# michael-fonder/M4Depth

Measured on AMD Instinct MI355X. Metric: frames/s, higher is better.
Workload: dtype f32

## Files before the change

include/m4depth_hip.h:

```cpp
#ifndef M4DEPTH_HIP_H_
#define M4DEPTH_HIP_H_

#include <stdint.h>

#ifdef __cplusplus
extern "C" {
#endif

#define M4D_ABI_VERSION 6

int m4d_abi_version(void);
long long m4d_launch_count(void);
const char* m4d_build_info(void);


int m4d_backproject_fwd(const float* input, const float* coords, const int dims[6],
                        float* out, void* stream);

int m4d_backproject_bwd(const float* grad, const float* input, const float* coords,
                        const int dims[6], float* input_grad, float* coords_grad, void* stream);


int m4d_dense_image_warp(const float* image, const float* flow, int B, int H, int W, int C,
                         float* out, int32_t* index_out, void* stream);
// ... 196 lines not shown

int m4d_level_post(const float* refiner_out, const float* rot, int rot_c, const float* trans,
                   const float* cam_f, const float* cam_c, int b, int h, int w, float scale,
                   float* parallax, float* depth, float* other, float* depth_state, void* stream);

int m4d_bias_act(const float* x, const float* bias, long long rows, int C, float slope,
                 float* out, void* stream);

int m4d_bias_act_padded(const float* x, const float* bias, int b, int h, int w, int C, float slope,
                        float* out, int out_h, int out_w, int off_y, int off_x, void* stream);

int m4d_conv3x3_bias_act(const float* x, const float* wp, const float* bias, int b, int h, int w,
                         int Cin, int Cout, int CoutPad, float slope, float* out, void* stream);
long long m4d_conv3x3_workspace_floats(int b, int h, int w, int CoutPad);
int m4d_conv3x3s_bias_act_ws(const float* x, const float* wp, const float* bias, int b, int h, int w,
                             int Cin, int Cout, int CoutPad, int stride, float slope, float* out,
                             float* workspace, long long workspace_floats, void* stream);
int m4d_conv3x3_bias_act_ws(const float* x, const float* wp, const float* bias, int b, int h, int w,
                            int Cin, int Cout, int CoutPad, float slope, float* out, float* workspace,
                            long long workspace_floats, void* stream);
int m4d_conv3x3s_bias_act_wsb(const float* x, const float* wp, const float* bias, int b, int split_batch, int h, int w,
                              int Cin, int Cout, int CoutPad, int stride, float slope, float* out,
                              float* workspace, long long workspace_floats, void* stream);
int m4d_conv3x3_lat(const float* x, int s_in, long long x_slab_floats, const float* x_bias, float x_slope,
                    const void* wp, const float* bias, int b, int h, int w, int Cin, int Cout, float slope,
                    int mt, int kw, int s_out, float* out, long long out_slab_floats, void* stream);
int m4d_conv3x3s_lat(const float* x, int s_in, long long x_slab_floats, const float* x_bias, float x_slope,
                     const void* wp, const float* bias, int b, int h, int w, int Cin, int Cout, int stride, float slope,
                     int mt, int kw, int s_out, float* out, long long out_slab_floats, void* stream);
int m4d_conv3x3_lat_f16(const float* x, int s_in, long long x_slab_floats, const float* x_bias, float x_slope,
                        const void* wp, const float* bias, int b, int h, int w, int Cin, int Cout, float slope,
                        int mt, int kw, int s_out, float* out, long long out_slab_floats, void* stream);
int m4d_partial_finish(const float* x, int s_in, long long x_slab_floats, const float* bias, float slope,
                       long long pixels, int C, float* out, void* stream);

int m4d_conv3x3_small_bias_act(const float* x, const float* wp, const float* bias, int b, int h, int w,
                               int Cin, int Cout, int CoutPad, float slope, float* out, void* stream);
int m4d_conv3x3s_small_bias_act(const float* x, const float* wp, const float* bias, int b, int h, int w,
                                int Cin, int Cout, int CoutPad, int stride, float slope, float* out, void* stream);
int m4d_conv3x3_small6_bias_act(const float* x, const void* wp6, const float* bias, int b, int h, int w,
                                int Cin, int Cout, int CoutPad, float slope, float* out, void* stream);

long long m4d_dinl_workspace_floats(int b, int C);
int m4d_dinl_fwd_padded(const float* x, const float* scale, const float* bias, int b, int h, int w, int C,
                        float slope, float* workspace, float* out, int out_h, int out_w, int off_y,
                        int off_x, void* stream);
int m4d_dinl_fwd(const float* x, const float* scale, const float* bias, int b, int h, int w, int C,
                 float slope, float* workspace, float* out, void* stream);

int m4d_enc_level0_fwd(const float* images, int bsz, long long stride_b, long long stride_t,
                       const float* w1_hwio, const float* bias1, const float* dn_scale, const float* dn_bias,
                       float dn_slope, const float* w2_hwio, const float* bias2, float slope,
                       int b, int h, int w, float* workspace, float* out, void* stream);
int m4d_enc_level0_stats(const float* images, int bsz, long long stride_b, long long stride_t,
                         const float* w1_hwio, const float* bias1, int b, int h, int w, float* workspace,
                         float* mean, float* var, void* stream);
int m4d_enc_level0_apply(const float* images, int bsz, long long stride_b, long long stride_t,
                         const float* w1_hwio, const float* bias1, const float* mean, const float* var,
                         const float* dn_scale, const float* dn_bias, float dn_slope, const float* w2_hwio,
                         const float* bias2, float slope, int b, int h, int w, float* out, void* stream);
int m4d_enc_head_fwd(const float* images, int bsz, long long stride_b, long long stride_t,
                     const float* w_hwio, const float* bias, int b, int h, int w, int C,
// ... 60 lines not shown
```

m4depth_amd/_lib.py:

```python
from __future__ import annotations

import ctypes
import os

import torch

_HERE = os.path.dirname(os.path.abspath(__file__))
LIB_FLAVOUR = os.environ.get("M4D_LIB_FLAVOUR", "product")
LIB_PATH = os.path.join(_HERE, "libm4depth_hip_exp.so" if LIB_FLAVOUR == "experiments" else "libm4depth_hip.so")

ABI_VERSION = 6

_c_fp = ctypes.c_void_p
_c_int = ctypes.c_int
_c_f = ctypes.c_float

class NormLevel(ctypes.Structure):
    _fields_ = [("x", ctypes.c_void_p), ("out", ctypes.c_void_p), ("pixels", ctypes.c_longlong), ("C", ctypes.c_int),
                ("nbre_cuts", ctypes.c_int)]


class ResetLevel(ctypes.Structure):
    _fields_ = [("features", ctypes.c_void_p), ("state_features", ctypes.c_void_p), ("depth_state", ctypes.c_void_p),
                ("parallax", ctypes.c_void_p), ("depth", ctypes.c_void_p), ("other", ctypes.c_void_p),
# ... 42 lines not shown
    "m4d_depth_export": [_c_fp, ctypes.c_longlong, _c_fp, ctypes.c_longlong, _c_fp, ctypes.c_longlong, _c_int, _c_int, _c_int,
                         _c_int, _c_fp, _c_int, ctypes.POINTER(_c_int), _c_fp, _c_f, _c_f, _c_f, _c_fp, _c_fp],
    "m4d_pose_accumulate": [_c_fp, _c_int, _c_fp, _c_fp, _c_int, _c_fp, _c_fp],
    "m4d_depth_cloud": [_c_fp, ctypes.c_longlong, _c_fp, ctypes.c_longlong, _c_fp, _c_fp, _c_fp, _c_int, _c_int, _c_int, _c_int,
                        _c_f, _c_f, _c_fp, _c_fp, _c_fp, _c_fp],
    "m4d_summary_images": [_c_int, ctypes.POINTER(ctypes.c_void_p), ctypes.POINTER(ctypes.c_longlong), ctypes.POINTER(_c_int),
                           ctypes.POINTER(_c_int), ctypes.POINTER(_c_int), ctypes.POINTER(_c_int),
                           ctypes.POINTER(ctypes.c_longlong), _c_int, _c_fp, _c_fp],
    "m4d_normalize_cuts": [_c_fp, _c_int, _c_int, _c_int, _c_int, _c_int, _c_fp, _c_fp],
    "m4d_resize_bilinear_v1": [_c_fp, _c_int, _c_int, _c_int, _c_int, _c_int, _c_int, _c_f, _c_fp, _c_fp],
    "m4d_resize_nearest": [_c_fp, _c_int, _c_int, _c_int, _c_int, _c_int, _c_int, _c_fp, _c_fp],
    "m4d_bias_act": [_c_fp, _c_fp, ctypes.c_longlong, _c_int, _c_f, _c_fp, _c_fp],
    "m4d_dinl_fwd": [_c_fp, _c_fp, _c_fp, _c_int, _c_int, _c_int, _c_int, _c_f, _c_fp, _c_fp, _c_fp],
    "m4d_dinl_fwd_padded": [_c_fp, _c_fp, _c_fp, _c_int, _c_int, _c_int, _c_int, _c_f, _c_fp, _c_fp,
                            _c_int, _c_int, _c_int, _c_int, _c_fp],
    "m4d_bias_act_padded": [_c_fp, _c_fp, _c_int, _c_int, _c_int, _c_int, _c_f, _c_fp, _c_int, _c_int, _c_int, _c_int, _c_fp],
    "m4d_conv3x3_bias_act": [_c_fp, _c_fp, _c_fp, _c_int, _c_int, _c_int, _c_int, _c_int, _c_int, _c_f, _c_fp, _c_fp],
    "m4d_conv3x3_bias_act_ws": [_c_fp, _c_fp, _c_fp, _c_int, _c_int, _c_int, _c_int, _c_int, _c_int, _c_f, _c_fp,
                                _c_fp, ctypes.c_longlong, _c_fp],
    "m4d_conv3x3s_bias_act_ws": [_c_fp, _c_fp, _c_fp, _c_int, _c_int, _c_int, _c_int, _c_int, _c_int, _c_int, _c_f,
                                 _c_fp, _c_fp, ctypes.c_longlong, _c_fp],
    "m4d_conv3x3s_bias_act_wsb": [_c_fp, _c_fp, _c_fp, _c_int, _c_int, _c_int, _c_int, _c_int, _c_int, _c_int, _c_int, _c_f,
                                  _c_fp, _c_fp, ctypes.c_longlong, _c_fp],
    "m4d_conv3x3_small_bias_act": [_c_fp, _c_fp, _c_fp, _c_int, _c_int, _c_int, _c_int, _c_int, _c_int, _c_f, _c_fp, _c_fp],
    "m4d_conv3x3s_small_bias_act": [_c_fp, _c_fp, _c_fp, _c_int, _c_int, _c_int, _c_int, _c_int, _c_int, _c_int, _c_f, _c_fp, _c_fp],
    "m4d_conv3x3_small6_bias_act": [_c_fp, _c_fp, _c_fp, _c_int, _c_int, _c_int, _c_int, _c_int, _c_int, _c_f, _c_fp, _c_fp],
    "m4d_conv3x3_lat": [_c_fp, _c_int, ctypes.c_longlong, _c_fp, _c_f, _c_fp, _c_fp, _c_int, _c_int, _c_int, _c_int, _c_int, _c_f,
                        _c_int, _c_int, _c_int, _c_fp, ctypes.c_longlong, _c_fp],
    "m4d_conv3x3s_lat": [_c_fp, _c_int, ctypes.c_longlong, _c_fp, _c_f, _c_fp, _c_fp, _c_int, _c_int, _c_int, _c_int, _c_int, _c_int,
                         _c_f, _c_int, _c_int, _c_int, _c_fp, ctypes.c_longlong, _c_fp],
    "m4d_conv3x3_lat_f16": [_c_fp, _c_int, ctypes.c_longlong, _c_fp, _c_f, _c_fp, _c_fp, _c_int, _c_int, _c_int, _c_int, _c_int,
                            _c_f, _c_int, _c_int, _c_int, _c_fp, ctypes.c_longlong, _c_fp],
    "m4d_partial_finish": [_c_fp, _c_int, ctypes.c_longlong, _c_fp, _c_f, ctypes.c_longlong, _c_int, _c_fp, _c_fp],
    "m4d_conv3x3_wino_bias_act": [_c_fp, _c_fp, _c_fp, _c_int, _c_int, _c_int, _c_int, _c_int, _c_int, _c_f, _c_fp, _c_fp],
    "m4d_conv3x3_wino2_bias_act": [_c_fp, _c_fp, _c_fp, _c_int, _c_int, _c_int, _c_int, _c_int, _c_int, _c_f, _c_fp, _c_fp],
    "m4d_conv3x3_wino6_bias_act": [_c_fp, _c_fp, _c_fp, _c_int, _c_int, _c_int, _c_int, _c_int, _c_int, _c_f, _c_fp, _c_fp],
    "m4d_conv3x3_wino6_bias_act_k": [_c_fp, _c_fp, _c_fp, _c_int, _c_int, _c_int, _c_int, _c_int, _c_int, _c_f, _c_fp, _c_int, _c_fp],
    "m4d_conv3x3_wino6_bias_act_ks": [_c_fp, _c_fp, _c_fp, _c_int, _c_int, _c_int, _c_int, _c_int, _c_int, _c_f, _c_fp, _c_int,
                                      _c_int, _c_int, _c_fp],
    "m4d_conv3x3_winof16_bias_act_ks": [_c_fp, _c_fp, _c_fp, _c_int, _c_int, _c_int, _c_int, _c_int, _c_int, _c_f, _c_fp,
                                        _c_int, _c_int, _c_fp],
    "m4d_enc_head_fwd": [_c_fp, _c_int, ctypes.c_longlong, ctypes.c_longlong, _c_fp, _c_fp, _c_int, _c_int, _c_int, _c_int,
                         _c_fp, _c_fp, _c_fp],
    "m4d_enc_level0_stats": [_c_fp, _c_int, ctypes.c_longlong, ctypes.c_longlong, _c_fp, _c_fp, _c_int, _c_int, _c_int, _c_fp, _c_fp, _c_fp,
                             _c_fp],
    "m4d_enc_level0_apply": [_c_fp, _c_int, ctypes.c_longlong, ctypes.c_longlong, _c_fp, _c_fp, _c_fp, _c_fp, _c_fp, _c_fp, _c_f, _c_fp,
                             _c_fp, _c_f, _c_int, _c_int, _c_int, _c_fp, _c_fp],
    "m4d_enc_level0_fwd": [_c_fp, _c_int, ctypes.c_longlong, ctypes.c_longlong, _c_fp, _c_fp, _c_fp, _c_fp, _c_f, _c_fp, _c_fp, _c_f,
# ... 171 lines not shown
```

m4depth_amd/csrc/m4d_conv.hip:

```cpp
#include <cstdlib>
#include "m4d_common.h"
#include "../../include/m4depth_hip.h"

namespace {

typedef float f32x16 __attribute__((ext_vector_type(16)));

struct ConvArgs {
  const float* x; const float* wp; const float* bias; float* out;
  int b, h, w, Cin, Cout, CoutPad, n_chunks, tiles_x, tiles_y;
  int oh, ow, pad_y, pad_x;
  float slope;
  int ksplit, chunks_per_split;
  float* ws;
  const float* dn_mean; const float* dn_var; const float* dn_scale; const float* dn_bias; float dn_slope;
  int ablate;
};

constexpr int kTW = 16, kTH = 8;
constexpr int kKC = 16, kRS = 20;

template <int NT, int TS, int STRIDE, bool DB, int MINB, bool DINL = false>
__global__ void __launch_bounds__(256, MINB)
conv3x3_mfma_kernel(const ConvArgs a) {
// ... 580 lines not shown
void dispatch_conv(const ConvArgs& a, int nt, dim3 grid, hipStream_t s) {
  const long long blocks = (long long)grid.x * grid.y * grid.z;
  static long long occ3_min_blocks = -1;
  if (occ3_min_blocks < 0) { const char* e = getenv("M4D_CONV_OCC3_MIN_BLOCKS"); occ3_min_blocks = e ? atoll(e) : 4 * 768; }
  switch (nt) {
    case 4:
      if (STRIDE == 1 && blocks >= occ3_min_blocks) launch_conv<4, 3, STRIDE, STRIDE == 1 ? 3 : 1>(a, grid, s);
      else launch_conv<4, 3, STRIDE, STRIDE == 1 ? 2 : 1>(a, grid, s);
      break;
    case 3: launch_conv<3, 3, STRIDE, STRIDE == 1 ? 3 : 2>(a, grid, s); break;
    case 2: launch_conv<2, STRIDE == 1 ? 9 : 3, STRIDE, STRIDE == 1 ? 3 : 2>(a, grid, s); break;
    default: launch_conv<1, 9, STRIDE, STRIDE == 1 ? 4 : 2>(a, grid, s); break;
  }
}

}

extern "C" int m4d_conv3x3_bias_act(const float* x, const float* wp, const float* bias, int b, int h, int w,
                                    int Cin, int Cout, int CoutPad, float slope, float* out, void* stream) {
  return m4d_conv3x3s_bias_act_ws(x, wp, bias, b, h, w, Cin, Cout, CoutPad, 1, slope, out, nullptr, 0, stream);
}

static int launch_conv3x3_small(const float* x, const float* wp, const float* bias, int b, int h, int w, int Cin, int Cout,
                                int CoutPad, int stride, float slope, float* out, void* stream) {
  M4D_CHECK_ARG(x && wp && bias && out && b > 0 && h > 0 && w > 0 && Cout > 0 && (stride == 1 || stride == 2));
  M4D_CHECK_ARG(Cin >= 16 && Cin % 4 == 0 && CoutPad % 32 == 0 && CoutPad >= Cout);
  M4D_CHECK_ARG(((((uintptr_t)x) | ((uintptr_t)wp)) & 15u) == 0);
  ConvArgs a;
  a.x = x; a.wp = wp; a.bias = bias; a.out = out; a.b = b; a.h = h; a.w = w; a.Cin = Cin; a.Cout = Cout;
  a.CoutPad = CoutPad; a.n_chunks = (Cin + kKC - 1) / kKC;
  a.dn_mean = a.dn_var = a.dn_scale = a.dn_bias = nullptr; a.dn_slope = 1.0f;
  a.ablate = 0; a.slope = slope;
  a.oh = (h + stride - 1) / stride; a.ow = (w + stride - 1) / stride;
  const int tot_y = (a.oh - 1) * stride + 3 - h, tot_x = (a.ow - 1) * stride + 3 - w;
  a.pad_y = (tot_y > 0 ? tot_y : 0) / 2; a.pad_x = (tot_x > 0 ? tot_x : 0) / 2;
  a.tiles_x = (a.ow + kSW - 1) / kSW; a.tiles_y = (a.oh + kSH - 1) / kSH;
  a.ksplit = 1; a.chunks_per_split = a.n_chunks; a.ws = nullptr;
  const int halo = ((kSW - 1) * stride + 3) * ((kSH - 1) * stride + 3);
  const size_t lds = (size_t)4 * (halo * kRS + kSB) * sizeof(float);
  if (stride == 1) M4D_LDS_OPT_IN(&conv3x3_small_kernel<1>);
  else M4D_LDS_OPT_IN(&conv3x3_small_kernel<2>);
  const dim3 grid((unsigned)(a.tiles_x * a.tiles_y), (unsigned)(CoutPad / 32), (unsigned)b);
  if (stride == 1) m4d_launch(conv3x3_small_kernel<1>, grid, dim3(256), lds, (hipStream_t)stream, a);
  else m4d_launch(conv3x3_small_kernel<2>, grid, dim3(256), lds, (hipStream_t)stream, a);
  return M4D_LAUNCH_RESULT();
}
extern "C" int m4d_conv3x3_small_bias_act(const float* x, const float* wp, const float* bias, int b, int h, int w,
                                          int Cin, int Cout, int CoutPad, float slope, float* out, void* stream) {
  return launch_conv3x3_small(x, wp, bias, b, h, w, Cin, Cout, CoutPad, 1, slope, out, stream);
}
extern "C" int m4d_conv3x3s_small_bias_act(const float* x, const float* wp, const float* bias, int b, int h, int w,
                                           int Cin, int Cout, int CoutPad, int stride, float slope, float* out, void* stream) {
  return launch_conv3x3_small(x, wp, bias, b, h, w, Cin, Cout, CoutPad, stride, slope, out, stream);
}

extern "C" int m4d_conv3x3_small6_bias_act(const float* x, const void* wp6, const float* bias, int b, int h, int w,
                                           int Cin, int Cout, int CoutPad, float slope, float* out, void* stream) {
  M4D_CHECK_ARG(x && wp6 && bias && out && b > 0 && h > 0 && w > 0 && Cout > 0);
  M4D_CHECK_ARG(Cin >= 16 && Cin % 4 == 0 && CoutPad % 32 == 0 && CoutPad >= Cout);
  M4D_CHECK_ARG(((((uintptr_t)x) | ((uintptr_t)wp6)) & 15u) == 0);
  ConvArgs a;
  a.x = x; a.wp = reinterpret_cast<const float*>(wp6); a.bias = bias; a.out = out; a.b = b; a.h = h; a.w = w; a.Cin = Cin; a.Cout = Cout;
  a.CoutPad = CoutPad; a.n_chunks = (Cin + kKC - 1) / kKC;
  a.dn_mean = a.dn_var = a.dn_scale = a.dn_bias = nullptr; a.dn_slope = 1.0f;
  a.ablate = 0; a.oh = h; a.ow = w; a.pad_y = a.pad_x = 1; a.slope = slope;
  a.tiles_x = (w + kSW - 1) / kSW; a.tiles_y = (h + kSH - 1) / kSH;
  a.ksplit = 1; a.chunks_per_split = a.n_chunks; a.ws = nullptr;
  constexpr size_t lds = (size_t)4 * (kS6A + kS6B) * sizeof(float);
  M4D_LDS_OPT_IN(&conv3x3_small6_kernel);
  m4d_launch(conv3x3_small6_kernel, dim3((unsigned)(a.tiles_x * a.tiles_y), (unsigned)(CoutPad / 32), (unsigned)b), dim3(256),
                     lds, (hipStream_t)stream, a);
  return M4D_LAUNCH_RESULT();
}

extern "C" long long m4d_conv3x3_workspace_floats(int b, int h, int w, int CoutPad) {
  return 32LL * b * h * w * CoutPad;
// ... 23 lines not shown
  a.dn_mean = mean; a.dn_var = var; a.dn_scale = dn_scale; a.dn_bias = dn_bias; a.dn_slope = dn_slope;
  constexpr int HP = ((kTW - 1) * 2 + 3) * ((kTH - 1) * 2 + 3);
  constexpr size_t lds = (size_t)(HP * kRS + 9 * 32 * kRS) * sizeof(float);
  if (lds > 64 * 1024) M4D_LDS_OPT_IN(&conv3x3_mfma_kernel<1, 9, 2, false, 2, true>);
  const dim3 grid((unsigned)(a.tiles_x * a.tiles_y), 1, (unsigned)b);
  m4d_launch((conv3x3_mfma_kernel<1, 9, 2, false, 2, true>), grid, dim3(256), lds, (hipStream_t)stream, a);
  return M4D_LAUNCH_RESULT();
}

extern "C" int m4d_conv3x3s_bias_act_wsb(const float* x, const float* wp, const float* bias, int b, int split_batch, int h,
                                         int w, int Cin, int Cout, int CoutPad, int stride, float slope, float* out,
                                         float* workspace, long long workspace_floats, void* stream);

extern "C" int m4d_conv3x3s_bias_act_ws(const float* x, const float* wp, const float* bias, int b, int h, int w,
                                        int Cin, int Cout, int CoutPad, int stride, float slope, float* out,
                                        float* workspace, long long workspace_floats, void* stream) {
  return m4d_conv3x3s_bias_act_wsb(x, wp, bias, b, b, h, w, Cin, Cout, CoutPad, stride, slope, out, workspace,
                                   workspace_floats, stream);
}

extern "C" int m4d_conv3x3s_bias_act_wsb(const float* x, const float* wp, const float* bias, int b, int split_batch, int h,
                                         int w, int Cin, int Cout, int CoutPad, int stride, float slope, float* out,
                                         float* workspace, long long workspace_floats, void* stream) {
  M4D_CHECK_ARG(x && wp && bias && out && b > 0 && split_batch > 0 && h > 0 && w > 0 && Cin > 0 && Cout > 0);
  M4D_CHECK_ARG((stride == 1 || stride == 2) && CoutPad % 32 == 0 && CoutPad >= Cout);
  M4D_CHECK_ARG(((((uintptr_t)x) & (Cin % 2 == 0 ? 7u : 3u)) == 0) && ((((uintptr_t)wp) & 15u) == 0));
  ConvArgs a;
  a.x = x; a.wp = wp; a.bias = bias; a.out = out; a.b = b; a.h = h; a.w = w; a.Cin = Cin; a.Cout = Cout;
  a.CoutPad = CoutPad; a.n_chunks = (Cin + kKC - 1) / kKC;
  a.dn_mean = a.dn_var = a.dn_scale = a.dn_bias = nullptr; a.dn_slope = 1.0f;
  static int ablate = -1;
  if (ablate < 0) { const char* e = getenv("M4D_CONV_ABLATE"); ablate = e ? atoi(e) : 0; }
  a.ablate = ablate;
  a.oh = (h + stride - 1) / stride; a.ow = (w + stride - 1) / stride;
  const int tph = (a.oh - 1) * stride + 3 - h, tpw = (a.ow - 1) * stride + 3 - w;
  a.pad_y = (tph > 0 ? tph : 0) / 2; a.pad_x = (tpw > 0 ? tpw : 0) / 2;
  a.tiles_x = (a.ow + kTW - 1) / kTW; a.tiles_y = (a.oh + kTH - 1) / kTH; a.slope = slope;
  const long long tiles = (long long)a.tiles_x * a.tiles_y;
  const int n32 = CoutPad / 32;
  auto n_tiles_for = [&](int images) {
    int nt = n32 >= 4 && n32 % 4 == 0 ? 4 : (n32 % 3 == 0 ? 3 : (n32 % 2 == 0 ? 2 : 1));
    while (nt > 1 && tiles * images * (n32 / nt) < 512) nt = (nt == 4 || nt == 2) ? nt / 2 : 1;
    return nt;
  };
  const int nt = n_tiles_for(b);
  const long long blocks = tiles * split_batch * (n32 / n_tiles_for(split_batch));
  int ksplit = 1;
  static int sk_target = -1, sk_min_chunks = -1, sk_max = -1;
  if (sk_target < 0) { const char* e = getenv("M4D_CONV_SPLITK_TARGET"); sk_target = e ? atoi(e) : 256; }
  if (sk_min_chunks < 0) { const char* e = getenv("M4D_CONV_SPLITK_MIN_CHUNKS"); sk_min_chunks = e ? atoi(e) : 2; }
  if (sk_max < 0) { const char* e = getenv("M4D_CONV_SPLITK_MAX"); sk_max = e ? atoi(e) : 16; }
  if (workspace != nullptr && blocks < 128 && a.n_chunks >= 4) {
    ksplit = (int)((sk_target + blocks - 1) / blocks);
    if (ksplit > a.n_chunks / sk_min_chunks) ksplit = a.n_chunks / sk_min_chunks;
    if (ksplit > sk_max) ksplit = sk_max;
    while (ksplit > 1 && (long long)ksplit * b * a.oh * a.ow * CoutPad > workspace_floats) --ksplit;
  }
  a.chunks_per_split = (a.n_chunks + ksplit - 1) / ksplit;
  ksplit = (a.n_chunks + a.chunks_per_split - 1) / a.chunks_per_split;
  a.ksplit = ksplit; a.ws = workspace;
  const dim3 grid((unsigned)tiles, (unsigned)(n32 / nt), (unsigned)(b * ksplit));
  hipStream_t s = (hipStream_t)stream;
  if (stride == 1) dispatch_conv<1>(a, nt, grid, s);
  else dispatch_conv<2>(a, nt, grid, s);
  if (ksplit > 1) {
    const long long pixels = (long long)b * a.oh * a.ow;
    long long g = (pixels * Cout + 255) / 256;
    if (g > 2048) g = 2048;
    m4d_launch(conv_splitk_reduce_kernel, dim3((unsigned)g), dim3(256), 0, s, workspace, bias, pixels, Cout,
                       CoutPad, ksplit, slope, out);
  }
  return M4D_LAUNCH_RESULT();
}
```

m4depth_amd/network_ops.py:

```python
from __future__ import annotations

import ctypes

import torch

from ._lib import lib, dptr, stream_ptr, check, as_f32
from .depth_operations import _CV_ACCUM


def normalize_cuts(x, nbre_cuts, out=None):
    x = as_f32(x, "x")
    b, h, w, C = x.shape
    if C % nbre_cuts != 0:
        raise ValueError(f"nbre_cuts={nbre_cuts} does not divide the {C} feature channels")
    if out is None:
        out = torch.empty_like(x)
    check(lib.m4d_normalize_cuts(dptr(x, "x"), b, h, w, C, int(nbre_cuts), dptr(out, "out"), stream_ptr()),
          "m4d_normalize_cuts")
    return out


def resize_bilinear_v1(x, out_h, out_w, mul=1.0):
    x = as_f32(x, "x")
    b, ih, iw, c = x.shape
# ... 477 lines not shown
    for name, t in (("counter", counter), ("first_bad", first_bad)):
        if not isinstance(t, torch.Tensor) or t.numel() != 1:
            raise ValueError(f"{name}: expected a one-element int64 device tensor")
    ws = _workspace("train_log", int(lib.m4d_train_log_workspace_bytes()), est.device)
    check(lib.m4d_train_log_step(dptr(loss.reshape(1), "loss"), ctypes.c_void_p(gt.data_ptr()), gs, dptr(est, "est"), b, H, W,
                                 h, w, dptr(log, "log"), log.shape[0], dptr(counter, "counter", torch.int64),
                                 dptr(first_bad, "first_bad", torch.int64), dptr(ws), stream_ptr()), "m4d_train_log_step")
    return log

def pack_conv_weights(kernel_hwio):
    import numpy as np
    k = np.asarray(kernel_hwio, dtype=np.float32)
    assert k.shape[:2] == (3, 3)
    cin, cout = k.shape[2], k.shape[3]
    nch = -(-cin // 16)
    cpad = -(-cout // 32) * 32
    full = np.zeros((3, 3, nch * 16, cpad), np.float32)
    full[:, :, :cin, :cout] = k
    perm = np.array([0, 2, 4, 6, 8, 10, 12, 14, 1, 3, 5, 7, 9, 11, 13, 15])
    w = full.reshape(9, nch, 16, cpad)[:, :, perm, :]
    return np.ascontiguousarray(w.transpose(1, 0, 3, 2)), cpad


def conv3x3_bias_act(x, wp, bias, cout, cout_pad, slope=0.1, stride=1, split_batch=None):
    x = as_f32(x, "x")
    b, h, w, cin = x.shape
    split_b = b if split_batch is None else int(split_batch)
    oh, ow = -(-h // stride), -(-w // stride)
    out = torch.empty((b, oh, ow, cout), dtype=torch.float32, device=x.device)
    ws = None
    ws_floats = 0
    if split_b * oh * ow <= 16384:
        ws_floats = int(lib.m4d_conv3x3_workspace_floats(b, oh, ow, int(cout_pad)))
        ws = _workspace("conv_splitk", 4 * ws_floats, x.device)
    if split_batch is None:
        check(lib.m4d_conv3x3s_bias_act_ws(dptr(x, "x"), dptr(wp, "wp"), dptr(bias, "bias"), b, h, w, cin, int(cout),
                                           int(cout_pad), int(stride), float(slope), dptr(out), dptr(ws), ws_floats,
                                           stream_ptr()), "m4d_conv3x3s_bias_act_ws")
    else:
        check(lib.m4d_conv3x3s_bias_act_wsb(dptr(x, "x"), dptr(wp, "wp"), dptr(bias, "bias"), b, split_b, h, w, cin, int(cout),
                                            int(cout_pad), int(stride), float(slope), dptr(out), dptr(ws), ws_floats,
                                            stream_ptr()), "m4d_conv3x3s_bias_act_wsb")
    return out


def conv3x3_small_bias_act(x, wp, bias, cout, cout_pad, slope=0.1, stride=1):
    x = as_f32(x, "x")
    b, h, w, cin = x.shape
    out = torch.empty((b, -(-h // stride), -(-w // stride), cout), dtype=torch.float32, device=x.device)
    check(lib.m4d_conv3x3s_small_bias_act(dptr(x, "x"), dptr(wp, "wp"), dptr(bias, "bias"), b, h, w, cin, int(cout),
                                          int(cout_pad), int(stride), float(slope), dptr(out), stream_ptr()),
          "m4d_conv3x3s_small_bias_act")
    return out


_WINO_G = [[1.0, 0.0, 0.0], [0.5, 0.5, 0.5], [0.5, -0.5, 0.5], [0.0, 0.0, 1.0]]


_WINO_SKEW = 64


def pack_conv_weights_winograd(kernel_hwio, chunk=16):
    import numpy as np
    k = np.asarray(kernel_hwio, dtype=np.float64)
    assert k.shape[:2] == (3, 3)
    cin, cout = k.shape[2], k.shape[3]
    G = np.array(_WINO_G, np.float64)
    U = np.einsum('ij,jkco,lk->ilco', G, k, G)
    nch = -(-cin // chunk)
    cpad = -(-cout // 32) * 32
    full = np.zeros((16, nch * chunk, cpad), np.float32)
    full[:, :cin, :cout] = U.reshape(16, cin, cout).astype(np.float32)
    w = np.ascontiguousarray(full.reshape(16, nch, chunk, cpad).transpose(1, 0, 3, 2))
    if chunk == 8:
        skewed = np.zeros((nch, 16, cpad * chunk + _WINO_SKEW), np.float32)
# ... 549 lines not shown
```

Measured before the change: 1793.

## Add dedicated stride-2 conv3x3 MFMA kernels with auto-dispatch

Adds a new stride-2 3x3 convolution implementation with two kernels. One is a pipelined, multi-tile-per-workgroup MFMA kernel with double-buffered halo and weight staging in LDS. The other is a small-shape kernel that splits input-channel chunks across waves and reduces the partial sums in LDS. The default dispatch now sends all stride-2 small convs, and stride-2 regular convs meeting a heuristic, to the new kernels, which aims to cut wasted work and improve occupancy on downsampling layers. The heuristic thresholds are hand-picked and the new code adds correctness risk.

New measurement: 1792. No clear change (-0.1%).

```diff
diff --git a/include/m4depth_hip.h b/include/m4depth_hip.h
--- a/include/m4depth_hip.h
+++ b/include/m4depth_hip.h
@@ -242,6 +242,9 @@
 int m4d_conv3x3s_bias_act_wsb(const float* x, const float* wp, const float* bias, int b, int split_batch, int h, int w,
                               int Cin, int Cout, int CoutPad, int stride, float slope, float* out,
                               float* workspace, long long workspace_floats, void* stream);
+int m4d_conv3x3s_bias_act_wsb_k(const float* x, const float* wp, const float* bias, int b, int split_batch, int h, int w,
+                                int Cin, int Cout, int CoutPad, int stride, float slope, float* out,
+                                float* workspace, long long workspace_floats, int kernel, void* stream);
 int m4d_conv3x3_lat(const float* x, int s_in, long long x_slab_floats, const float* x_bias, float x_slope,
                     const void* wp, const float* bias, int b, int h, int w, int Cin, int Cout, float slope,
                     int mt, int kw, int s_out, float* out, long long out_slab_floats, void* stream);
@@ -258,6 +261,8 @@
                                int Cin, int Cout, int CoutPad, float slope, float* out, void* stream);
 int m4d_conv3x3s_small_bias_act(const float* x, const float* wp, const float* bias, int b, int h, int w,
                                 int Cin, int Cout, int CoutPad, int stride, float slope, float* out, void* stream);
+int m4d_conv3x3s_small_bias_act_k(const float* x, const float* wp, const float* bias, int b, int h, int w,
+                                  int Cin, int Cout, int CoutPad, int stride, float slope, float* out, int kernel, void* stream);
 int m4d_conv3x3_small6_bias_act(const float* x, const void* wp6, const float* bias, int b, int h, int w,
                                 int Cin, int Cout, int CoutPad, float slope, float* out, void* stream);
 
diff --git a/m4depth_amd/_lib.py b/m4depth_amd/_lib.py
--- a/m4depth_amd/_lib.py
+++ b/m4depth_amd/_lib.py
@@ -88,8 +88,12 @@
                                  _c_fp, _c_fp, ctypes.c_longlong, _c_fp],
     "m4d_conv3x3s_bias_act_wsb": [_c_fp, _c_fp, _c_fp, _c_int, _c_int, _c_int, _c_int, _c_int, _c_int, _c_int, _c_int, _c_f,
                                   _c_fp, _c_fp, ctypes.c_longlong, _c_fp],
+    "m4d_conv3x3s_bias_act_wsb_k": [_c_fp, _c_fp, _c_fp, _c_int, _c_int, _c_int, _c_int, _c_int, _c_int, _c_int, _c_int, _c_f,
+                                    _c_fp, _c_fp, ctypes.c_longlong, _c_int, _c_fp],
     "m4d_conv3x3_small_bias_act": [_c_fp, _c_fp, _c_fp, _c_int, _c_int, _c_int, _c_int, _c_int, _c_int, _c_f, _c_fp, _c_fp],
     "m4d_conv3x3s_small_bias_act": [_c_fp, _c_fp, _c_fp, _c_int, _c_int, _c_int, _c_int, _c_int, _c_int, _c_int, _c_f, _c_fp, _c_fp],
+    "m4d_conv3x3s_small_bias_act_k": [_c_fp, _c_fp, _c_fp, _c_int, _c_int, _c_int, _c_int, _c_int, _c_int, _c_int, _c_f, _c_fp,
+                                      _c_int, _c_fp],
     "m4d_conv3x3_small6_bias_act": [_c_fp, _c_fp, _c_fp, _c_int, _c_int, _c_int, _c_int, _c_int, _c_int, _c_f, _c_fp, _c_fp],
     "m4d_conv3x3_lat": [_c_fp, _c_int, ctypes.c_longlong, _c_fp, _c_f, _c_fp, _c_fp, _c_int, _c_int, _c_int, _c_int, _c_int, _c_f,
                         _c_int, _c_int, _c_int, _c_fp, ctypes.c_longlong, _c_fp],
diff --git a/m4depth_amd/csrc/m4d_conv.hip b/m4depth_amd/csrc/m4d_conv.hip
--- a/m4depth_amd/csrc/m4d_conv.hip
+++ b/m4depth_amd/csrc/m4d_conv.hip
@@ -1,5 +1,6 @@
 #include <cstdlib>
 #include "m4d_common.h"
+#include "m4d_conv_s2.h"
 #include "../../include/m4depth_hip.h"
 
 namespace {
@@ -626,9 +627,10 @@
 }
 
 static int launch_conv3x3_small(const float* x, const float* wp, const float* bias, int b, int h, int w, int Cin, int Cout,
-                                int CoutPad, int stride, float slope, float* out, void* stream) {
+                                int CoutPad, int stride, float slope, float* out, int kernel, void* stream) {
   M4D_CHECK_ARG(x && wp && bias && out && b > 0 && h > 0 && w > 0 && Cout > 0 && (stride == 1 || stride == 2));
   M4D_CHECK_ARG(Cin >= 16 && Cin % 4 == 0 && CoutPad % 32 == 0 && CoutPad >= Cout);
+  M4D_CHECK_ARG(kernel >= 0 && kernel <= 2 && (kernel != 2 || stride == 2));
   M4D_CHECK_ARG(((((uintptr_t)x) | ((uintptr_t)wp)) & 15u) == 0);
   ConvArgs a;
   a.x = x; a.wp = wp; a.bias = bias; a.out = out; a.b = b; a.h = h; a.w = w; a.Cin = Cin; a.Cout = Cout;
@@ -640,6 +642,15 @@
   a.pad_y = (tot_y > 0 ? tot_y : 0) / 2; a.pad_x = (tot_x > 0 ? tot_x : 0) / 2;
   a.tiles_x = (a.ow + kSW - 1) / kSW; a.tiles_y = (a.oh + kSH - 1) / kSH;
   a.ksplit = 1; a.chunks_per_split = a.n_chunks; a.ws = nullptr;
+  if (kernel == 2 || (kernel == 0 && stride == 2)) {
+    M4dConvS2Args a2;
+    a2.x = x; a2.wp = wp; a2.bias = bias; a2.out = out; a2.ws = nullptr; a2.b = b; a2.h = h; a2.w = w; a2.Cin = Cin;
+    a2.Cout = Cout; a2.CoutPad = CoutPad; a2.n_chunks = a.n_chunks; a2.oh = a.oh; a2.ow = a.ow; a2.pad_y = a.pad_y;
+    a2.pad_x = a.pad_x; a2.ksplit = 1; a2.chunks_per_split = a.n_chunks; a2.slope = slope;
+    a2.tiles_x = a2.tiles_y = a2.tiles_per_wg = 0; a2.ablate = 0;
+    m4d_conv_s2_small_launch(a2, (hipStream_t)stream);
+    return M4D_LAUNCH_RESULT();
+  }
   const int halo = ((kSW - 1) * stride + 3) * ((kSH - 1) * stride + 3);
   const size_t lds = (size_t)4 * (halo * kRS + kSB) * sizeof(float);
   if (stride == 1) M4D_LDS_OPT_IN(&conv3x3_small_kernel<1>);
@@ -651,11 +662,16 @@
 }
 extern "C" int m4d_conv3x3_small_bias_act(const float* x, const float* wp, const float* bias, int b, int h, int w,
                                           int Cin, int Cout, int CoutPad, float slope, float* out, void* stream) {
-  return launch_conv3x3_small(x, wp, bias, b, h, w, Cin, Cout, CoutPad, 1, slope, out, stream);
+  return launch_conv3x3_small(x, wp, bias, b, h, w, Cin, Cout, CoutPad, 1, slope, out, 0, stream);
 }
 extern "C" int m4d_conv3x3s_small_bias_act(const float* x, const float* wp, const float* bias, int b, int h, int w,
                                            int Cin, int Cout, int CoutPad, int stride, float slope, float* out, void* stream) {
-  return launch_conv3x3_small(x, wp, bias, b, h, w, Cin, Cout, CoutPad, stride, slope, out, stream);
+  return launch_conv3x3_small(x, wp, bias, b, h, w, Cin, Cout, CoutPad, stride, slope, out, 0, stream);
+}
+extern "C" int m4d_conv3x3s_small_bias_act_k(const float* x, const float* wp, const float* bias, int b, int h, int w,
+                                             int Cin, int Cout, int CoutPad, int stride, float slope, float* out, int kernel,
+                                             void* stream) {
+  return launch_conv3x3_small(x, wp, bias, b, h, w, Cin, Cout, CoutPad, stride, slope, out, kernel, stream);
 }
 
 extern "C" int m4d_conv3x3_small6_bias_act(const float* x, const void* wp6, const float* bias, int b, int h, int w,
@@ -725,6 +741,14 @@
 extern "C" int m4d_conv3x3s_bias_act_wsb(const float* x, const float* wp, const float* bias, int b, int split_batch, int h,
                                          int w, int Cin, int Cout, int CoutPad, int stride, float slope, float* out,
                                          float* workspace, long long workspace_floats, void* stream) {
+  return m4d_conv3x3s_bias_act_wsb_k(x, wp, bias, b, split_batch, h, w, Cin, Cout, CoutPad, stride, slope, out, workspace,
+                                     workspace_floats, 0, stream);
+}
+
+extern "C" int m4d_conv3x3s_bias_act_wsb_k(const float* x, const float* wp, const float* bias, int b, int split_batch, int h,
+                                           int w, int Cin, int Cout, int CoutPad, int stride, float slope, float* out,
+                                           float* workspace, long long workspace_floats, int kernel, void* stream) {
+  M4D_CHECK_ARG(kernel >= 0 && kernel <= 2);
   M4D_CHECK_ARG(x && wp && bias && out && b > 0 && split_batch > 0 && h > 0 && w > 0 && Cin > 0 && Cout > 0);
   M4D_CHECK_ARG((stride == 1 || stride == 2) && CoutPad % 32 == 0 && CoutPad >= Cout);
   M4D_CHECK_ARG(((((uintptr_t)x) & (Cin % 2 == 0 ? 7u : 3u)) == 0) && ((((uintptr_t)wp) & 15u) == 0));
@@ -764,7 +788,17 @@
   a.ksplit = ksplit; a.ws = workspace;
   const dim3 grid((unsigned)tiles, (unsigned)(n32 / nt), (unsigned)(b * ksplit));
   hipStream_t s = (hipStream_t)stream;
-  if (stride == 1) dispatch_conv<1>(a, nt, grid, s);
+  M4dConvS2Args a2;
+  a2.x = x; a2.wp = wp; a2.bias = bias; a2.out = out; a2.ws = workspace; a2.b = b; a2.h = h; a2.w = w; a2.Cin = Cin;
+  a2.Cout = Cout; a2.CoutPad = CoutPad; a2.n_chunks = a.n_chunks; a2.oh = a.oh; a2.ow = a.ow; a2.pad_y = a.pad_y;
+  a2.pad_x = a.pad_x; a2.ksplit = ksplit; a2.chunks_per_split = a.chunks_per_split; a2.slope = slope;
+  a2.tiles_x = a2.tiles_y = a2.tiles_per_wg = 0; a2.ablate = ablate;
+  const bool s2_ok = stride == 2 && m4d_conv_s2_can_run(a2);
+  M4D_CHECK_ARG(kernel != 2 || s2_ok);
+  const bool s2_pays = s2_ok && ksplit == 1 && a.n_chunks <= 4 && n_tiles_for(split_batch) == 1 &&
+                       tiles * split_batch * n32 >= 128 && tiles * split_batch * n32 <= 1024;
+  if (kernel == 2 || (kernel == 0 && s2_pays)) m4d_conv_s2_launch(a2, s);
+  else if (stride == 1) dispatch_conv<1>(a, nt, grid, s);
   else dispatch_conv<2>(a, nt, grid, s);
   if (ksplit > 1) {
     const long long pixels = (long long)b * a.oh * a.ow;
diff --git a/m4depth_amd/csrc/m4d_conv_s2.h b/m4depth_amd/csrc/m4d_conv_s2.h
--- /dev/null
+++ b/m4depth_amd/csrc/m4d_conv_s2.h
@@ -0,0 +1,17 @@
+#pragma once
+#include <hip/hip_runtime.h>
+
+struct M4dConvS2Args {
+  const float* x; const float* wp; const float* bias; float* out;
+  float* ws;
+  int b, h, w, Cin, Cout, CoutPad, n_chunks;
+  int oh, ow, pad_y, pad_x;
+  int ksplit, chunks_per_split;
+  int tiles_x, tiles_y, tiles_per_wg;
+  float slope;
+  int ablate;
+};
+
+bool m4d_conv_s2_can_run(const M4dConvS2Args& a);
+void m4d_conv_s2_launch(M4dConvS2Args a, hipStream_t stream);
+void m4d_conv_s2_small_launch(M4dConvS2Args a, hipStream_t stream);
diff --git a/m4depth_amd/csrc/m4d_conv_s2.hip b/m4depth_amd/csrc/m4d_conv_s2.hip
--- /dev/null
+++ b/m4depth_amd/csrc/m4d_conv_s2.hip
@@ -0,0 +1,323 @@
+#include "m4d_common.h"
+#include "m4d_conv_s2.h"
+
+namespace {
+
+typedef float f32x16 __attribute__((ext_vector_type(16)));
+
+constexpr int kKC = 16, kRS = 20;
+constexpr int kTW = 16, kTH = 8;
+constexpr int kHW = (kTW - 1) * 2 + 3, kHH = (kTH - 1) * 2 + 3, kHP = kHW * kHH;
+constexpr int kThreads = 256;
+constexpr int kAF4 = kHP * 8;
+constexpr int kAPer = (kAF4 + kThreads - 1) / kThreads;
+constexpr int kBRows = 2 * 9 * 32;
+constexpr int kBPer = kBRows * 4 / kThreads;
+constexpr int kLdsA = 2 * kHP * kRS, kLdsB = kBRows * kRS;
+constexpr size_t kLds = (size_t)(kLdsA + kLdsB) * sizeof(float);
+
+template <bool ONE_PAIR>
+__global__ void __launch_bounds__(kThreads, 1)
+conv3x3_s2_kernel(const M4dConvS2Args a) {
+  extern __shared__ __align__(16) float lds_dyn[];
+  float* lds_a = lds_dyn;
+  float* lds_b = lds_dyn + kLdsA;
+  const int t = threadIdx.x, lane = t & 63, wave = t >> 6;
+  const int n0 = blockIdx.y * 32;
+  const int bi = blockIdx.z / a.ksplit, ks = blockIdx.z - bi * a.ksplit;
+  const int chunk_lo = ks * a.chunks_per_split;
+  const int chunk_hi = min(chunk_lo + a.chunks_per_split, a.n_chunks);
+  const int n_pairs = ONE_PAIR ? 1 : (chunk_hi - chunk_lo + 1) >> 1;
+  const int tile_lo = blockIdx.x * a.tiles_per_wg;
+  const int n_tiles = min(a.tiles_per_wg, a.tiles_x * a.tiles_y - tile_lo);
+  const int n_stages = n_tiles * n_pairs;
+  const float* ximg = a.x + (long long)bi * a.h * a.w * a.Cin;
+
+  const int pj = t & 7;
+  float4 ra[kAPer];
+  auto load_a = [&](int tile, int pair) __attribute__((always_inline)) {
+    const int ty = (tile / a.tiles_x) * kTH * 2 - a.pad_y, tx = (tile % a.tiles_x) * kTW * 2 - a.pad_x;
+    const int cc = min((chunk_lo + 2 * pair) * kKC + 4 * pj, a.Cin - 4);
+#pragma unroll
+    for (int u = 0; u < kAPer; ++u) {
+      const int hp = min((u * kThreads + t) >> 3, kHP - 1);
+      const int gy = ty + hp / kHW, gx = tx + hp % kHW;
+      const int off = (min(max(gy, 0), a.h - 1) * a.w + min(max(gx, 0), a.w - 1)) * a.Cin + cc;
+      ra[u] = *reinterpret_cast<const float4*>(ximg + off);
+    }
+  };
+  auto commit_a = [&](int tile, int pair) __attribute__((always_inline)) {
+    const int ty = (tile / a.tiles_x) * kTH * 2 - a.pad_y, tx = (tile % a.tiles_x) * kTW * 2 - a.pad_x;
+    const bool ch_ok = chunk_lo + 2 * pair + (pj >> 2) < chunk_hi;
+    float* dst0 = lds_a + (pj >> 2) * (kHP * kRS) + 2 * (pj & 3);
+#pragma unroll
+    for (int u = 0; u < kAPer; ++u) {
+      const int hp = (u * kThreads + t) >> 3;
+      const int gy = ty + hp / kHW, gx = tx + hp % kHW;
+      const bool ok = ch_ok && gy >= 0 && gy < a.h && gx >= 0 && gx < a.w;
+      const float4 v = ra[u];
+      if (hp < kHP) {
+        *reinterpret_cast<float2*>(dst0 + hp * kRS) = make_float2(ok ? v.x : 0.f, ok ? v.z : 0.f);
+        *reinterpret_cast<float2*>(dst0 + hp * kRS + 8) = make_float2(ok ? v.y : 0.f, ok ? v.w : 0.f);
+      }
+    }
+  };
+  float4 rb[kBPer];
+  auto load_b = [&](int pair) __attribute__((always_inline)) {
+#pragma unroll
+    for (int u = 0; u < kBPer; ++u) {
+      const int idx = u * kThreads + t, row = idx >> 2, c4 = idx & 3;
+      const int chunk = min(chunk_lo + 2 * pair + row / 288, chunk_hi - 1);
+      rb[u] = *reinterpret_cast<const float4*>(
+          a.wp + (((long long)chunk * 9 + (row % 288) / 32) * a.CoutPad + n0 + (row & 31)) * kKC + c4 * 4);
+    }
+  };
+  auto commit_b = [&]() __attribute__((always_inline)) {
+#pragma unroll
+    for (int u = 0; u < kBPer; ++u) {
+      const int idx = u * kThreads + t;
+      const float4 v = rb[u];
+      *reinterpret_cast<float4*>(lds_b + (idx >> 2) * kRS + (idx & 3) * 4) = make_float4(v.x, v.y, v.z, v.w);
+    }
+  };
+
+  f32x16 acc;
+#pragma unroll
+  for (int r = 0; r < 16; ++r) acc[r] = 0.f;
+  const int m = lane & 31, kh = lane >> 5;
+  const int prow = 2 * wave + (m >> 4), pcol = m & 15;
+  const float* a_lane = lds_a + (prow * 2 * kHW + pcol * 2) * kRS + kh * 8;
+  const float* b_lane = lds_b + m * kRS + kh * 8;
+  const int co = n0 + m;
+  const float bias = co < a.Cout ? a.bias[co] : 0.f;
+
+  struct Frag { float4 a0, a1, b0, b1; };
+  auto read_frag = [&](int half, int tap, Frag& f) __attribute__((always_inline)) {
+    const float* ap = a_lane + half * (kHP * kRS) + ((tap / 3) * kHW + (tap % 3)) * kRS;
+    const float* bp = b_lane + (half * 9 + tap) * 32 * kRS;
+    f.a0 = *reinterpret_cast<const float4*>(ap); f.a1 = *reinterpret_cast<const float4*>(ap + 4);
+    f.b0 = *reinterpret_cast<const float4*>(bp); f.b1 = *reinterpret_cast<const float4*>(bp + 4);
+  };
+  auto compute_half = [&](int half) __attribute__((always_inline)) {
+    Frag f[2];
+    read_frag(half, 0, f[0]);
+#pragma unroll
+    for (int tap = 0; tap < 9; ++tap) {
+      if (tap + 1 < 9) read_frag(half, tap + 1, f[(tap + 1) & 1]);
+      const Frag& g = f[tap & 1];
+      const float av[8] = {g.a0.x, g.a0.y, g.a0.z, g.a0.w, g.a1.x, g.a1.y, g.a1.z, g.a1.w};
+      const float bv[8] = {g.b0.x, g.b0.y, g.b0.z, g.b0.w, g.b1.x, g.b1.y, g.b1.z, g.b1.w};
+      if (!(a.ablate & 2)) {
+#pragma unroll
+        for (int k = 0; k < 8; ++k) acc = __builtin_amdgcn_mfma_f32_32x32x2f32(av[k], bv[k], acc, 0, 0, 0);
+      }
+    }
+  };
+  auto finish_tile = [&](int tile) __attribute__((always_inline)) {
+    const int tile_y = (tile / a.tiles_x) * kTH, tile_x = (tile % a.tiles_x) * kTW;
+    const bool skip = (a.ablate & 4) && acc[0] != 1.2345e-30f;
+#pragma unroll
+    for (int r = 0; r < 16; ++r) {
+      const int mr = (r & 3) + 8 * (r >> 2) + 4 * kh;
+      const int oy = tile_y + 2 * wave + (mr >> 4), ox = tile_x + (mr & 15);
+      if (oy < a.oh && ox < a.ow && !skip) {
+        if (a.ksplit > 1) {
+          a.ws[((((long long)ks * a.b + bi) * a.oh + oy) * a.ow + ox) * a.CoutPad + co] = acc[r];
+        } else if (co < a.Cout) {
+          float v = acc[r] + bias;
+          v = v > 0.f ? v : v * a.slope;
+          a.out[(((long long)bi * a.oh + oy) * a.ow + ox) * a.Cout + co] = v;
+        }
+      }
+      acc[r] = 0.f;
+    }
+  };
+  auto compute_stage = [&](int pair) __attribute__((always_inline)) {
+    compute_half(0);
+    if (chunk_lo + 2 * pair + 1 < chunk_hi) compute_half(1);
+  };
+
+  load_a(tile_lo, 0);
+  load_b(0);
+  commit_a(tile_lo, 0);
+  commit_b();
+  __syncthreads();
+  int tile = tile_lo, pair = 0;
+  for (int s = 0; s + 1 < n_stages; ++s) {
+    int ntile = tile, npair = pair + 1;
+    if (ONE_PAIR || npair == n_pairs) { npair = 0; ++ntile; }
+    load_a(ntile, npair);
+    if (!ONE_PAIR) load_b(npair);
+    compute_stage(pair);
+    __syncthreads();
+    commit_a(ntile, npair);
+    if (!ONE_PAIR) commit_b();
+    if (ONE_PAIR || npair == 0) finish_tile(tile);
+    __syncthreads();
+    tile = ntile; pair = npair;
+  }
+  compute_stage(pair);
+  finish_tile(tile);
+}
+
+constexpr int kSW = 8, kSH = 4;
+constexpr int kSHW = (kSW - 1) * 2 + 3, kSHH = (kSH - 1) * 2 + 3, kSHP = kSHW * kSHH;
+constexpr int kSA = kSHP * kRS;
+constexpr int kSAPer = (kSHP * 4 + 63) / 64;
+
+__global__ void __launch_bounds__(256, 2)
+conv3x3_s2_small_kernel(const M4dConvS2Args a) {
+  extern __shared__ __align__(16) float lds_dyn[];
+  const int t = threadIdx.x, lane = t & 63;
+  const int wave = __builtin_amdgcn_readfirstlane(t >> 6);
+  float* lds_a = lds_dyn + wave * kSA;
+  const int tile = blockIdx.x;
+  const int tile_y = (tile / a.tiles_x) * kSH, tile_x = (tile % a.tiles_x) * kSW;
+  const int n0 = blockIdx.y * 32;
+  const int bi = blockIdx.z;
+  const float* ximg = a.x + (long long)bi * a.h * a.w * a.Cin;
+
+  int a_off[kSAPer], a_dst[kSAPer];
+  unsigned a_ok = 0;
+  const int aq = lane & 3;
+#pragma unroll
+  for (int u = 0; u < kSAPer; ++u) {
+    const int idx = u * 64 + lane;
+    const int hp = min(idx >> 2, kSHP - 1);
+    const int gy = tile_y * 2 - a.pad_y + hp / kSHW, gx = tile_x * 2 - a.pad_x + hp % kSHW;
+    const bool ok = (idx >> 2) < kSHP && gy >= 0 && gy < a.h && gx >= 0 && gx < a.w;
+    a_ok |= ok ? (1u << u) : 0u;
+    a_off[u] = (min(max(gy, 0), a.h - 1) * a.w + min(max(gx, 0), a.w - 1)) * a.Cin + 4 * aq;
+    a_dst[u] = (idx >> 2) < kSHP ? hp * kRS + 2 * aq : -1;
+  }
+  float4 ra[kSAPer];
+  bool ra_ch_ok = true;
+  auto load_halo = [&](int chunk) __attribute__((always_inline)) {
+    const int c0 = chunk * kKC;
+    ra_ch_ok = c0 + 4 * aq < a.Cin;
+    const int cc = min(c0, a.Cin - 4 - 4 * aq);
+#pragma unroll
+    for (int u = 0; u < kSAPer; ++u) ra[u] = *reinterpret_cast<const float4*>(ximg + a_off[u] + cc);
+  };
+  auto commit_halo = [&]() __attribute__((always_inline)) {
+#pragma unroll
+    for (int u = 0; u < kSAPer; ++u) {
+      const bool ok = ((a_ok >> u) & 1u) && ra_ch_ok;
+      const float4 v = ra[u];
+      if (a_dst[u] >= 0) {
+        *reinterpret_cast<float2*>(lds_a + a_dst[u]) = make_float2(ok ? v.x : 0.f, ok ? v.z : 0.f);
+        *reinterpret_cast<float2*>(lds_a + a_dst[u] + 8) = make_float2(ok ? v.y : 0.f, ok ? v.w : 0.f);
+      }
+    }
+  };
+  const int m = lane & 31, kh = lane >> 5;
+  const float* wlane = a.wp + (long long)(n0 + m) * kKC + kh * 8;
+  const long long wtap = (long long)a.CoutPad * kKC;
+  float4 rb[9][2];
+  auto load_b_tap = [&](int chunk, int tap) __attribute__((always_inline)) {
+    const float* p = wlane + ((long long)chunk * 9 + tap) * wtap;
+    rb[tap][0] = *reinterpret_cast<const float4*>(p);
+    rb[tap][1] = *reinterpret_cast<const float4*>(p + 4);
+  };
+
+  f32x16 acc;
+#pragma unroll
+  for (int r = 0; r < 16; ++r) acc[r] = 0.f;
+  const float* a_lane = lds_a + ((m >> 3) * 2 * kSHW + (m & 7) * 2) * kRS + kh * 8;
+  auto compute_chunk = [&](int next_chunk) __attribute__((always_inline)) {
+#pragma unroll
+    for (int tap = 0; tap < 9; ++tap) {
+      const float* ap = a_lane + ((tap / 3) * kSHW + (tap % 3)) * kRS;
+      const float4 a0 = *reinterpret_cast<const float4*>(ap), a1 = *reinterpret_cast<const float4*>(ap + 4);
+      const float4 b0 = rb[tap][0], b1 = rb[tap][1];
+      const float av[8] = {a0.x, a0.y, a0.z, a0.w, a1.x, a1.y, a1.z, a1.w};
+      const float bv[8] = {b0.x, b0.y, b0.z, b0.w, b1.x, b1.y, b1.z, b1.w};
+#pragma unroll
+      for (int k = 0; k < 8; ++k) acc = __builtin_amdgcn_mfma_f32_32x32x2f32(av[k], bv[k], acc, 0, 0, 0);
+      if (next_chunk >= 0) load_b_tap(next_chunk, tap);
+    }
+  };
+
+  if (wave < a.n_chunks) {
+    load_halo(wave);
+#pragma unroll
+    for (int tap = 0; tap < 9; ++tap) load_b_tap(wave, tap);
+    int c = wave;
+    for (; c + 4 < a.n_chunks; c += 4) {
+      commit_halo();
+      __builtin_amdgcn_wave_barrier();
+      load_halo(c + 4);
+      compute_chunk(c + 4);
+      __builtin_amdgcn_wave_barrier();
+    }
+    commit_halo();
+    __builtin_amdgcn_wave_barrier();
+    compute_chunk(-1);
+    __builtin_amdgcn_wave_barrier();
+  }
+  __syncthreads();
+
+  constexpr int kRP = 36;
+  float* red = lds_dyn;
+#pragma unroll
+  for (int r = 0; r < 16; ++r) {
+    const int mr = (r & 3) + 8 * (r >> 2) + 4 * kh;
+    red[(wave * 32 + mr) * kRP + m] = acc[r];
+  }
+  __syncthreads();
+  {
+    const int p = t >> 3, cq = t & 7;
+    const int oy = tile_y + (p >> 3), ox = tile_x + (p & 7);
+    const int co = n0 + 4 * cq;
+    if (oy < a.oh && ox < a.ow && co < a.Cout) {
+      const float4 s0 = *reinterpret_cast<const float4*>(red + (0 * 32 + p) * kRP + 4 * cq);
+      const float4 s1 = *reinterpret_cast<const float4*>(red + (1 * 32 + p) * kRP + 4 * cq);
+      const float4 s2 = *reinterpret_cast<const float4*>(red + (2 * 32 + p) * kRP + 4 * cq);
+      const float4 s3 = *reinterpret_cast<const float4*>(red + (3 * 32 + p) * kRP + 4 * cq);
+      const float sum[4] = {((s0.x + s1.x) + s2.x) + s3.x, ((s0.y + s1.y) + s2.y) + s3.y,
+                            ((s0.z + s1.z) + s2.z) + s3.z, ((s0.w + s1.w) + s2.w) + s3.w};
+      float* op = a.out + (((long long)bi * a.oh + oy) * a.ow + ox) * a.Cout + co;
+#pragma unroll
+      for (int e = 0; e < 4; ++e) {
+        if (co + e < a.Cout) {
+          float v = sum[e] + a.bias[co + e];
+          op[e] = v > 0.f ? v : v * a.slope;
+        }
+      }
+    }
+  }
+}
+
+}
+
+void m4d_conv_s2_small_launch(M4dConvS2Args a, hipStream_t stream) {
+  a.tiles_x = (a.ow + kSW - 1) / kSW;
+  a.tiles_y = (a.oh + kSH - 1) / kSH;
+  a.tiles_per_wg = 1;
+  const dim3 grid((unsigned)(a.tiles_x * a.tiles_y), (unsigned)(a.CoutPad / 32), (unsigned)a.b);
+  m4d_launch(conv3x3_s2_small_kernel, grid, dim3(256), (size_t)4 * kSA * sizeof(float), stream, a);
+}
+
+bool m4d_conv_s2_can_run(const M4dConvS2Args& a) {
+  return a.Cin >= kKC && a.Cin % kKC == 0 && a.Cout % 32 == 0 && a.CoutPad == a.Cout && ((((uintptr_t)a.x) & 15u) == 0) &&
+         (long long)a.h * a.w * a.Cin < (1LL << 31);
+}
+
+void m4d_conv_s2_launch(M4dConvS2Args a, hipStream_t stream) {
+  a.tiles_x = (a.ow + kTW - 1) / kTW;
+  a.tiles_y = (a.oh + kTH - 1) / kTH;
+  const long long tiles = (long long)a.tiles_x * a.tiles_y;
+  const long long units = tiles * (a.CoutPad / 32) * a.b * a.ksplit;
+  const int cus = m4d_device_cus() > 0 ? m4d_device_cus() : 256;
+  long long tpw = (units + cus - 1) / cus;
+  if (tpw > tiles) tpw = tiles;
+  a.tiles_per_wg = (int)(tpw < 1 ? 1 : tpw);
+  const dim3 grid((unsigned)((tiles + a.tiles_per_wg - 1) / a.tiles_per_wg), (unsigned)(a.CoutPad / 32), (unsigned)(a.b * a.ksplit));
+  if (a.chunks_per_split <= 2) {
+    M4D_LDS_OPT_IN(&conv3x3_s2_kernel<true>);
+    m4d_launch(conv3x3_s2_kernel<true>, grid, dim3(kThreads), kLds, stream, a);
+  } else {
+    M4D_LDS_OPT_IN(&conv3x3_s2_kernel<false>);
+    m4d_launch(conv3x3_s2_kernel<false>, grid, dim3(kThreads), kLds, stream, a);
+  }
+}
diff --git a/m4depth_amd/network_ops.py b/m4depth_amd/network_ops.py
--- a/m4depth_amd/network_ops.py
+++ b/m4depth_amd/network_ops.py
@@ -523,7 +523,7 @@
     return np.ascontiguousarray(w.transpose(1, 0, 3, 2)), cpad
 
 
-def conv3x3_bias_act(x, wp, bias, cout, cout_pad, slope=0.1, stride=1, split_batch=None):
+def conv3x3_bias_act(x, wp, bias, cout, cout_pad, slope=0.1, stride=1, split_batch=None, kernel=0):
     x = as_f32(x, "x")
     b, h, w, cin = x.shape
     split_b = b if split_batch is None else int(split_batch)
@@ -534,7 +534,11 @@
     if split_b * oh * ow <= 16384:
         ws_floats = int(lib.m4d_conv3x3_workspace_floats(b, oh, ow, int(cout_pad)))
         ws = _workspace("conv_splitk", 4 * ws_floats, x.device)
-    if split_batch is None:
+    if kernel:
+        check(lib.m4d_conv3x3s_bias_act_wsb_k(dptr(x, "x"), dptr(wp, "wp"), dptr(bias, "bias"), b, split_b, h, w, cin, int(cout),
+                                              int(cout_pad), int(stride), float(slope), dptr(out), dptr(ws), ws_floats,
+                                              int(kernel), stream_ptr()), "m4d_conv3x3s_bias_act_wsb_k")
+    elif split_batch is None:
         check(lib.m4d_conv3x3s_bias_act_ws(dptr(x, "x"), dptr(wp, "wp"), dptr(bias, "bias"), b, h, w, cin, int(cout),
                                            int(cout_pad), int(stride), float(slope), dptr(out), dptr(ws), ws_floats,
                                            stream_ptr()), "m4d_conv3x3s_bias_act_ws")
@@ -545,13 +549,13 @@
     return out
 
 
-def conv3x3_small_bias_act(x, wp, bias, cout, cout_pad, slope=0.1, stride=1):
+def conv3x3_small_bias_act(x, wp, bias, cout, cout_pad, slope=0.1, stride=1, kernel=0):
     x = as_f32(x, "x")
     b, h, w, cin = x.shape
     out = torch.empty((b, -(-h // stride), -(-w // stride), cout), dtype=torch.float32, device=x.device)
-    check(lib.m4d_conv3x3s_small_bias_act(dptr(x, "x"), dptr(wp, "wp"), dptr(bias, "bias"), b, h, w, cin, int(cout),
-                                          int(cout_pad), int(stride), float(slope), dptr(out), stream_ptr()),
-          "m4d_conv3x3s_small_bias_act")
+    check(lib.m4d_conv3x3s_small_bias_act_k(dptr(x, "x"), dptr(wp, "wp"), dptr(bias, "bias"), b, h, w, cin, int(cout),
+                                            int(cout_pad), int(stride), float(slope), dptr(out), int(kernel), stream_ptr()),
+          "m4d_conv3x3s_small_bias_act_k")
     return out
 
 
```
